# ActiveVisionLab/gaussctrl

Measured on AMD Instinct MI355X. Metric: edited views/sec @512x512 (ControlNet denoise + splat render+bwd), higher is better.
Workload: dtype bf16

## Files before the change

gaussctrl_amd/csrc/dn_gemm_kernels.h:

```cpp
#pragma once
#include "dn_common.h"
#include <type_traits>

namespace dng {
struct GemmArgs {
    int64_t M, N, K;
    const void *A; int64_t lda;
    int B, Hi, Wi, Cin, Ho, Wo, stride, ups, pad;
    const void *W;
    const float *bias;
    const float *rowvec; int64_t ld_rowvec; int64_t rows_per_batch;
    const void *residual; int64_t ldr;
    float out_scale;
    int act, geglu;
    void *out; int64_t ldc; int out_f32;
    void *out_t; int64_t ldt; int64_t t_batch_stride; int64_t t_col0;
    int splits; int tiles_per_split;
    int persist;
    float *ws;
    const void *zeros;
    const float *row_stats; int row_stat_slots; const float *colsum; float ln_eps, ln_inv_k;
    float *out_row_stats;
    float *out_group_stats;
    int gn_groups, gn_cpg;
    const unsigned char *w_scale;
    int a_scale;
    int out_fp8; float out_qscale;
    int dbg;
    float *chan_parts; int cp_nslab; int cp_rows;
    int64_t w_set_rows, w_set_stride;
    int pw;
    int sm_keys;
    int conv_korder;
};

__device__ __forceinline__ void tile_coords(int64_t bid, int nbm, int nbn, int pw, int64_t &mblk, int64_t &nblk)
{
    if (pw <= 0 || pw >= nbn) { mblk = bid / nbn; nblk = bid % nbn; return; }
    const int64_t per = (int64_t)nbm * pw, p = bid / per, within = bid - p * per;
    const int64_t w = (nbn - p * pw) < pw ? (nbn - p * pw) : pw;
    mblk = within / w; nblk = p * pw + within % w;
}
__device__ __forceinline__ void wg_tile(const GemmArgs &g, int nbm, int nbn, int64_t &mblk, int64_t &nblk, int &slice)
{
    const int64_t tiles = gridDim.x, total = tiles * gridDim.y, lin = blockIdx.x + tiles * blockIdx.y;
    const int64_t xcd = lin & 7, qq = total >> 3, rr = total & 7;
    const int64_t L = (xcd < rr ? xcd * (qq + 1) : rr * (qq + 1) + (xcd - rr) * qq) + (lin >> 3);
    slice = (int)(L / tiles);
    tile_coords(L - (int64_t)slice * tiles, nbm, nbn, g.pw, mblk, nblk);
}
}

namespace {
using namespace dn;
using dng::GemmArgs;

template <int I, int N, class F> __device__ __forceinline__ void static_for(F &&f)
{
    if constexpr (I < N) {
        f(std::integral_constant<int, I>{});
        static_for<I + 1, N>(f);
    }
}

constexpr int BM = 128, BK = 64;
constexpr int NT = 256;


constexpr int GS_SLOTS = 20, GS_MAXG = 32;

__device__ __forceinline__ float row16_sum(float v)
{
    v += __builtin_bit_cast(float, __builtin_amdgcn_update_dpp(0, __builtin_bit_cast(int, v), 0x128, 0xf, 0xf, false));
    v += __builtin_bit_cast(float, __builtin_amdgcn_update_dpp(0, __builtin_bit_cast(int, v), 0x124, 0xf, 0xf, false));
    v += __builtin_bit_cast(float, __builtin_amdgcn_update_dpp(0, __builtin_bit_cast(int, v), 0x122, 0xf, 0xf, false));
    v += __builtin_bit_cast(float, __builtin_amdgcn_update_dpp(0, __builtin_bit_cast(int, v), 0x121, 0xf, 0xf, false));
    return v;
}

__device__ __forceinline__ int lds_off(int r, int c) { return r * 128 + ((c ^ ((r >> 1) & 7)) << 4); }

template <class T>
__device__ __forceinline__ void epilogue_store(const GemmArgs &g, int64_t m, int64_t n, int64_t on, float *v, const float *gate, const uint2 *res_pre = nullptr)
{
    const int64_t bidx = g.rowvec ? m / g.rows_per_batch : 0;
    if (g.row_stats) {
        float2 rs = make_float2(0.f, 0.f);
        for (int sl = 0; sl < g.row_stat_slots; ++sl) {
            const float2 t = *reinterpret_cast<const float2 *>(g.row_stats + ((int64_t)sl * g.M + m) * 2);
            rs.x += t.x; rs.y += t.y;
        }
        const float mean = rs.x * g.ln_inv_k, rstd = rsqrtf(fmaxf(rs.y * g.ln_inv_k - mean * mean, 0.f) + g.ln_eps);
#pragma unroll
        for (int r = 0; r < 4; ++r) v[r] = rstd * (v[r] - mean * g.colsum[n + r]);
    }
#pragma unroll
    for (int r = 0; r < 4; ++r) {
        if (g.bias) v[r] += g.bias[n + r];
        if (g.rowvec) v[r] += g.rowvec[bidx * g.ld_rowvec + n + r];
    }
    if (g.geglu) {
#pragma unroll
        for (int r = 0; r < 4; ++r) {
            float gt = gate[r];
            if (g.bias) gt += g.bias[n + 16 + r];
            v[r] = v[r] * gelu_erf(gt);
        }
    }
    if (g.act == 1) {
#pragma unroll
        for (int r = 0; r < 4; ++r) v[r] = silu(v[r]);
    } else if (g.act == 2) {
#pragma unroll
        for (int r = 0; r < 4; ++r) v[r] = fminf(fmaxf(v[r] * 0.5f + 0.5f, 0.f), 1.f);
    }
#pragma unroll
    for (int r = 0; r < 4; ++r) v[r] *= g.out_scale;
    if (g.residual) {
        const uint2 rr = res_pre ? *res_pre : *reinterpret_cast<const uint2 *>((const unsigned char *)g.residual + (m * g.ldr + on) * 2);
        v[0] += T::to_f((unsigned short)(rr.x & 0xffff)); v[1] += T::to_f((unsigned short)(rr.x >> 16));
        v[2] += T::to_f((unsigned short)(rr.y & 0xffff)); v[3] += T::to_f((unsigned short)(rr.y >> 16));
    }
    const bool to_t = g.out_t && on >= g.t_col0;
    const uint2 pk = make_uint2(pack2<T>(v[0], v[1]), pack2<T>(v[2], v[3]));
    if (g.out && !(to_t && g.t_col0 > 0)) {
        if (g.out_f32)
            *reinterpret_cast<float4 *>((float *)g.out + m * g.ldc + on) = make_float4(v[0], v[1], v[2], v[3]);
        else
            *reinterpret_cast<uint2 *>((unsigned char *)g.out + (m * g.ldc + on) * 2) = pk;
    }
    if (to_t) {
        const int64_t b = m / g.rows_per_batch, tok = m - b * g.rows_per_batch;
        unsigned short *o = (unsigned short *)g.out_t + b * g.t_batch_stride + tok;
#pragma unroll
        for (int r = 0; r < 4; ++r) o[(on - g.t_col0 + r) * g.ldt] = T::from_f(v[r]);
    }
    if (!g.out_f32) {
        v[0] = T::to_f((unsigned short)(pk.x & 0xffff)); v[1] = T::to_f((unsigned short)(pk.x >> 16));
        v[2] = T::to_f((unsigned short)(pk.y & 0xffff)); v[3] = T::to_f((unsigned short)(pk.y >> 16));
    }
}

template <int BM>
__device__ __forceinline__ void row_stats_prologue(const GemmArgs &g, int64_t m_base, float *srow)
{
    const int t = threadIdx.x, r = t & 255, half = t >> 8;
    if (t < 2 * BM) srow[t] = 0.f;
    asm volatile("s_waitcnt lgkmcnt(0)" ::: "memory");
    __builtin_amdgcn_s_barrier();
    if (r < BM) {
        const int64_t m = m_base + r < g.M ? m_base + r : g.M - 1;
        const float *rp = g.row_stats + m * 2;
        const int64_t st = g.M * 2;
        float sx = 0.f, sy = 0.f;
        int sl = half;
        for (; sl + 6 < g.row_stat_slots; sl += 8) {
            const float2 a = *reinterpret_cast<const float2 *>(rp + sl * st), b = *reinterpret_cast<const float2 *>(rp + (sl + 2) * st);
            const float2 c = *reinterpret_cast<const float2 *>(rp + (sl + 4) * st), d = *reinterpret_cast<const float2 *>(rp + (sl + 6) * st);
            sx += (a.x + b.x) + (c.x + d.x); sy += (a.y + b.y) + (c.y + d.y);
        }
        for (; sl < g.row_stat_slots; sl += 2) {
            const float2 a = *reinterpret_cast<const float2 *>(rp + sl * st);
            sx += a.x; sy += a.y;
        }
        __hip_atomic_fetch_add(srow + 2 * r, sx, __ATOMIC_RELAXED, __HIP_MEMORY_SCOPE_WORKGROUP);
        __hip_atomic_fetch_add(srow + 2 * r + 1, sy, __ATOMIC_RELAXED, __HIP_MEMORY_SCOPE_WORKGROUP);
    }
    asm volatile("s_waitcnt vmcnt(0) lgkmcnt(0)" ::: "memory");
}

template <class T, int NTW, int MT, int NTHREADS>
__device__ __forceinline__ void wave_epilogue(const GemmArgs &g, f32x4 (&acc)[NTW][MT], int64_t m_base, int64_t m_wave, int64_t n_wave, int lane,
                                              unsigned char *smem, const float *srow = nullptr, int slice = 0)
{
    const int fr = lane & 15, fc = lane >> 4;
    const int64_t n_lane = n_wave + fc * 4;
    if (g.splits > 1) {
#pragma unroll
        for (int mt = 0; mt < MT; ++mt) {
            const int64_t m = m_wave + mt * 16 + fr;
            if (m >= g.M) continue;
#pragma unroll
            for (int nt = 0; nt < NTW; ++nt) {
                const int64_t n = n_lane + nt * 16;
                if (n < g.N)
                    *reinterpret_cast<float4 *>(g.ws + ((int64_t)slice * g.M + m) * g.N + n) =
                        make_float4(acc[nt][mt][0], acc[nt][mt][1], acc[nt][mt][2], acc[nt][mt][3]);
            }
        }
        return;
    }
    if (g.out_group_stats) {
        asm volatile("s_waitcnt lgkmcnt(0)" ::: "memory");
        __builtin_amdgcn_s_barrier();
        for (int idx = threadIdx.x; idx < GS_SLOTS * GS_MAXG * 2; idx += NTHREADS) reinterpret_cast<float *>(smem)[idx] = 0.f;
        asm volatile("s_waitcnt lgkmcnt(0)" ::: "memory");
        __builtin_amdgcn_s_barrier();
    }
    float4 bia[NTW], csm[NTW];
#pragma unroll
    for (int nt = 0; nt < NTW; ++nt) {
        const int64_t n = n_lane + nt * 16;
        bia[nt] = (g.bias && n < g.N) ? *reinterpret_cast<const float4 *>(g.bias + n) : make_float4(0.f, 0.f, 0.f, 0.f);
        csm[nt] = (g.row_stats && n < g.N) ? *reinterpret_cast<const float4 *>(g.colsum + n) : make_float4(0.f, 0.f, 0.f, 0.f);
    }
    uint2 rs_all[MT][NTW];
#pragma unroll
    for (int mt = 0; mt < MT; ++mt) {
        const int64_t m = m_wave + mt * 16 + fr;
        const bool okm = m < g.M;
        const int64_t mc = okm ? m : 0;
#pragma unroll
        for (int nt = 0; nt < NTW; ++nt) {
            const int64_t n = n_lane + nt * 16;
            const bool okn = okm && n < g.N && !(g.geglu && (nt & 1));
            const int64_t on = g.geglu ? (n_wave + nt * 16) / 2 + fc * 4 : n;
            rs_all[mt][nt] = (g.residual && okn) ? *reinterpret_cast<const uint2 *>((const unsigned char *)g.residual + (mc * g.ldr + on) * 2) : make_uint2(0u, 0u);
        }
    }
    const bool want_cs = g.out_group_stats != nullptr;
    float *red = reinterpret_cast<float *>(smem);
    const int64_t b0 = want_cs ? m_base / g.rows_per_batch : 0;
    float cs[NTW][4], css[NTW][4];
#pragma unroll
    for (int nt = 0; nt < NTW; ++nt)
#pragma unroll
        for (int r = 0; r < 4; ++r) { cs[nt][r] = 0.f; css[nt][r] = 0.f; }
    int64_t cs_b = -1;
    auto flush_cs = [&]() __attribute__((always_inline)) {
        float *rb = red + (cs_b - b0) * (GS_MAXG * 2);
#pragma unroll
        for (int nt = 0; nt < NTW; ++nt) {
            const int64_t n = n_lane + nt * 16;
#pragma unroll
            for (int r = 0; r < 4; ++r) {
                const float a = (g.dbg & 4) ? cs[nt][r] : row16_sum(cs[nt][r]), b = (g.dbg & 4) ? css[nt][r] : row16_sum(css[nt][r]);
                if (fr == 0 && n + r < g.N && !(g.dbg & 2)) {
                    const int gi = (int)(n + r) / g.gn_cpg;
                    __hip_atomic_fetch_add(rb + 2 * gi, a, __ATOMIC_RELAXED, __HIP_MEMORY_SCOPE_WORKGROUP);
                    __hip_atomic_fetch_add(rb + 2 * gi + 1, b, __ATOMIC_RELAXED, __HIP_MEMORY_SCOPE_WORKGROUP);
                }
                cs[nt][r] = 0.f; css[nt][r] = 0.f;
            }
        }
    };
#pragma unroll
    for (int mt = 0; mt < MT; ++mt) {
        const int64_t m = m_wave + mt * 16 + fr;
        const int64_t m_tile = m_wave + mt * 16;
        if (m_tile >= g.M) break;
        const bool okm = m < g.M;
        if (want_cs) {
            const int64_t b = m_tile / g.rows_per_batch;
            if (cs_b >= 0 && b != cs_b) flush_cs();
            cs_b = b;
        }
        const uint2 *rs = rs_all[mt];
        float mean = 0.f, rstd = 1.f;
        if (g.row_stats) {
            float sx = 0.f, sy = 0.f;
            if (srow) {
                const float2 t = *reinterpret_cast<const float2 *>(srow + 2 * (okm ? (int)(m - m_base) : 0));
                sx = t.x; sy = t.y;
            } else {
                const float *rp = g.row_stats + (okm ? m : 0) * 2;
                for (int sl = 0; sl < g.row_stat_slots; ++sl) {
                    const float2 t = *reinterpret_cast<const float2 *>(rp + (int64_t)sl * g.M * 2);
                    sx += t.x; sy += t.y;
                }
            }
            mean = sx * g.ln_inv_k;
            rstd = rsqrtf(fmaxf(sy * g.ln_inv_k - mean * mean, 0.f) + g.ln_eps);
        }
        float4 rv[NTW];
        const int64_t bidx = (g.rowvec && okm) ? m / g.rows_per_batch : 0;
#pragma unroll
        for (int nt = 0; nt < NTW; ++nt) {
            const int64_t n = n_lane + nt * 16;
            rv[nt] = (g.rowvec && n < g.N) ? *reinterpret_cast<const float4 *>(g.rowvec + bidx * g.ld_rowvec + n) : make_float4(0.f, 0.f, 0.f, 0.f);
        }
        float rsum = 0.f, rsq = 0.f;
#pragma unroll
        for (int nt = 0; nt < NTW; ++nt) {
            const int64_t n = n_lane + nt * 16;
            if (n >= g.N) continue;
            if (g.geglu && (nt & 1)) continue;
            float a0 = acc[nt][mt][0], a1 = acc[nt][mt][1], a2 = acc[nt][mt][2], a3 = acc[nt][mt][3];
            if (g.row_stats) {
                a0 = rstd * (a0 - mean * csm[nt].x); a1 = rstd * (a1 - mean * csm[nt].y);
                a2 = rstd * (a2 - mean * csm[nt].z); a3 = rstd * (a3 - mean * csm[nt].w);
            }
            float v[4] = {a0 + bia[nt].x + rv[nt].x, a1 + bia[nt].y + rv[nt].y, a2 + bia[nt].z + rv[nt].z, a3 + bia[nt].w + rv[nt].w};
            int64_t on = n;
            if (g.geglu) {
                constexpr int NP = NTW - 1;
                const int np = nt + 1 < NTW ? nt + 1 : NP;
                float g0 = acc[np][mt][0], g1 = acc[np][mt][1], g2 = acc[np][mt][2], g3 = acc[np][mt][3];
                if (g.row_stats) {
                    g0 = rstd * (g0 - mean * csm[np].x); g1 = rstd * (g1 - mean * csm[np].y);
                    g2 = rstd * (g2 - mean * csm[np].z); g3 = rstd * (g3 - mean * csm[np].w);
                }
                v[0] *= gelu_erf(g0 + bia[np].x); v[1] *= gelu_erf(g1 + bia[np].y);
                v[2] *= gelu_erf(g2 + bia[np].z); v[3] *= gelu_erf(g3 + bia[np].w);
                on = (n_wave + nt * 16) / 2 + fc * 4;
            }
            if (g.act == 1) {
#pragma unroll
                for (int r = 0; r < 4; ++r) v[r] = silu(v[r]);
            } else if (g.act == 2) {
#pragma unroll
                for (int r = 0; r < 4; ++r) v[r] = fminf(fmaxf(v[r] * 0.5f + 0.5f, 0.f), 1.f);
            }
#pragma unroll
            for (int r = 0; r < 4; ++r) v[r] *= g.out_scale;
            if (g.residual) {
                v[0] += T::to_f((unsigned short)(rs[nt].x & 0xffff)); v[1] += T::to_f((unsigned short)(rs[nt].x >> 16));
                v[2] += T::to_f((unsigned short)(rs[nt].y & 0xffff)); v[3] += T::to_f((unsigned short)(rs[nt].y >> 16));
// ... 728 lines not shown
                const uint2 pk = make_uint2(pack2<T>(v[0], v[1]), pack2<T>(v[2], v[3]));
                const bool ok = m < g.M && n < g.N;
                if (ok) *reinterpret_cast<uint2 *>((unsigned char *)g.out + (m * g.ldc + n) * 2) = pk;
                if constexpr (CS) pks[mt][nt] = ok ? pk : make_uint2(0u, 0u);
                if constexpr (LNV == 1) {
                    const float w_ = n < g.N ? 1.f : 0.f;
                    const float t0 = w_ * T::to_f((unsigned short)(pk.x & 0xffff)), t1 = w_ * T::to_f((unsigned short)(pk.x >> 16));
                    const float t2 = w_ * T::to_f((unsigned short)(pk.y & 0xffff)), t3 = w_ * T::to_f((unsigned short)(pk.y >> 16));
                    rsum += (t0 + t1) + (t2 + t3); rsq += (t0 * t0 + t1 * t1) + (t2 * t2 + t3 * t3);
                }
            }
            if constexpr (LNV == 1) {
                rsum += __shfl_xor(rsum, 16, 64); rsq += __shfl_xor(rsq, 16, 64);
                rsum += __shfl_xor(rsum, 32, 64); rsq += __shfl_xor(rsq, 32, 64);
                const int64_t slot = (n_base + wn * (16 * NTW)) / (16 * NTW);
                if (fc == 0 && m < g.M && n_base + wn * (16 * NTW) < g.N)
                    *reinterpret_cast<float2 *>(g.out_row_stats + (slot * g.M + m) * 2) = make_float2(rsum, rsq);
            }
        }
        if constexpr (CS) {
            const int64_t m_split = (m_base / g.rows_per_batch + 1) * g.rows_per_batch;
            const int64_t m_end = m_base + BM < g.M ? m_base + BM : g.M;
            const int npass = m_split < m_end ? 2 : 1;
    #pragma unroll 1
            for (int pass = 0; pass < npass; ++pass) {
                float cs[NTW][4], cq[NTW][4];
    #pragma unroll
                for (int nt = 0; nt < NTW; ++nt)
    #pragma unroll
                    for (int r = 0; r < 4; ++r) { cs[nt][r] = 0.f; cq[nt][r] = 0.f; }
    #pragma unroll
                for (int mt = 0; mt < MT; ++mt) {
                    const int64_t m_tile = m_base + wm * (16 * MT) + mt * 16;
                    const float wgt = ((m_tile >= m_split ? 1 : 0) == pass) ? 1.f : 0.f;
    #pragma unroll
                    for (int nt = 0; nt < NTW; ++nt) {
                        const uint2 pk = pks[mt][nt];
                        const float t0 = wgt != 0.f ? T::to_f((unsigned short)(pk.x & 0xffff)) : 0.f, t1 = wgt != 0.f ? T::to_f((unsigned short)(pk.x >> 16)) : 0.f;
                        const float t2 = wgt != 0.f ? T::to_f((unsigned short)(pk.y & 0xffff)) : 0.f, t3 = wgt != 0.f ? T::to_f((unsigned short)(pk.y >> 16)) : 0.f;
                        cs[nt][0] += t0; cq[nt][0] += t0 * t0; cs[nt][1] += t1; cq[nt][1] += t1 * t1;
                        cs[nt][2] += t2; cq[nt][2] += t2 * t2; cs[nt][3] += t3; cq[nt][3] += t3 * t3;
                    }
                }
                float *tb = ctab + (pass * BN + wn * (16 * NTW) + fc * 4) * 2;
    #pragma unroll
                for (int nt = 0; nt < NTW; ++nt)
    #pragma unroll
                    for (int r = 0; r < 4; ++r) {
                        const float sa = row16_sum(cs[nt][r]), sb = row16_sum(cq[nt][r]);
                        if (fr == 0) {
                            __hip_atomic_fetch_add(tb + (nt * 16 + r) * 2, sa, __ATOMIC_RELAXED, __HIP_MEMORY_SCOPE_WORKGROUP);
                            __hip_atomic_fetch_add(tb + (nt * 16 + r) * 2 + 1, sb, __ATOMIC_RELAXED, __HIP_MEMORY_SCOPE_WORKGROUP);
                        }
                    }
            }
            asm volatile("s_waitcnt lgkmcnt(0)" ::: "memory");
            __builtin_amdgcn_s_barrier();
            const int64_t b0 = m_base / g.rows_per_batch;
            const int cpg = g.gn_cpg, G = (int)(g.N / cpg);
            const int n_hi = (int)(n_base + BN < g.N ? n_base + BN : g.N);
            const int g_first = (int)n_base / cpg, ng = (n_hi - 1) / cpg - g_first + 1;
            for (int i = tid; i < 2 * ng; i += 512) {
                const int slot = i >= ng ? 1 : 0, gg = g_first + i - slot * ng;
                if (slot == 1 && !(m_split < m_end)) continue;
                const int c_lo = gg * cpg > (int)n_base ? gg * cpg : (int)n_base, c_hi = (gg + 1) * cpg < n_hi ? (gg + 1) * cpg : n_hi;
                float s1 = 0.f, s2 = 0.f;
                for (int c = c_lo; c < c_hi; ++c) { const float2 t = *reinterpret_cast<const float2 *>(ctab + (slot * BN + c - (int)n_base) * 2); s1 += t.x; s2 += t.y; }
                const int64_t b = b0 + slot;
                const int64_t slab = mblk - (b * g.rows_per_batch) / BM;
                const int half = gg * cpg < (int)n_base ? 1 : 0;
                *reinterpret_cast<float2 *>(g.chan_parts + ((((b * g.cp_nslab + slab) * G + gg) * 2 + half) * 2)) = make_float2(s1, s2);
            }
        }
    } else {
    float4 bia[NTW], csm[LNV == 2 ? NTW : 1];
#pragma unroll
    for (int nt = 0; nt < NTW; ++nt) {
        const int64_t n = n_lane + nt * 16;
        bia[nt] = (g.bias && n < g.N) ? *reinterpret_cast<const float4 *>(g.bias + n) : make_float4(0.f, 0.f, 0.f, 0.f);
        if constexpr (LNV == 2) csm[nt] = n < g.N ? *reinterpret_cast<const float4 *>(g.colsum + n) : make_float4(0.f, 0.f, 0.f, 0.f);
    }
#pragma unroll
    for (int mt = 0; mt < MT; ++mt) {
        const int64_t m = m_base + wm * (16 * MT) + mt * 16 + fr;
        if (m >= g.M) continue;
        if constexpr (LNV == 2) {
            const float2 st = *reinterpret_cast<const float2 *>(srow + 2 * (wm * (16 * MT) + mt * 16 + fr));
            const float mean = st.x * g.ln_inv_k, rstd = rsqrtf(fmaxf(st.y * g.ln_inv_k - mean * mean, 0.f) + g.ln_eps);
#pragma unroll
            for (int nt = 0; nt < NTW; ++nt) {
                acc[nt][mt][0] = rstd * (acc[nt][mt][0] - mean * csm[nt].x); acc[nt][mt][1] = rstd * (acc[nt][mt][1] - mean * csm[nt].y);
                acc[nt][mt][2] = rstd * (acc[nt][mt][2] - mean * csm[nt].z); acc[nt][mt][3] = rstd * (acc[nt][mt][3] - mean * csm[nt].w);
            }
        }
        float4 rv[NTW];
        uint2 rs[NTW];
        const int64_t bidx = g.rowvec ? m / g.rows_per_batch : 0;
#pragma unroll
        for (int nt = 0; nt < NTW; ++nt) {
            const int64_t n = n_lane + nt * 16;
            const bool okn = n < g.N && !(g.geglu && (nt & 1));
            const int64_t on = g.geglu ? (n_base + wn * (16 * NTW) + nt * 16) / 2 + fc * 4 : n;
            rv[nt] = (g.rowvec && n < g.N) ? *reinterpret_cast<const float4 *>(g.rowvec + bidx * g.ld_rowvec + n) : make_float4(0.f, 0.f, 0.f, 0.f);
            rs[nt] = (g.residual && okn) ? *reinterpret_cast<const uint2 *>((const unsigned char *)g.residual + (m * g.ldr + on) * 2) : make_uint2(0u, 0u);
        }
#pragma unroll
        for (int nt = 0; nt < NTW; ++nt) {
            const int64_t n = n_lane + nt * 16;
            if (n >= g.N) continue;
            if (g.geglu && (nt & 1)) continue;
            float v[4] = {acc[nt][mt][0] + bia[nt].x + rv[nt].x, acc[nt][mt][1] + bia[nt].y + rv[nt].y,
                          acc[nt][mt][2] + bia[nt].z + rv[nt].z, acc[nt][mt][3] + bia[nt].w + rv[nt].w};
            int64_t on = n;
            if (g.geglu) {
                constexpr int NP = NTW - 1;
                const int np = nt + 1 < NTW ? nt + 1 : NP;
                v[0] *= gelu_erf(acc[np][mt][0] + bia[np].x); v[1] *= gelu_erf(acc[np][mt][1] + bia[np].y);
                v[2] *= gelu_erf(acc[np][mt][2] + bia[np].z); v[3] *= gelu_erf(acc[np][mt][3] + bia[np].w);
                on = (n_base + wn * (16 * NTW) + nt * 16) / 2 + fc * 4;
            }
            if (g.act == 1) {
#pragma unroll
                for (int r = 0; r < 4; ++r) v[r] = silu(v[r]);
            } else if (g.act == 2) {
#pragma unroll
                for (int r = 0; r < 4; ++r) v[r] = fminf(fmaxf(v[r] * 0.5f + 0.5f, 0.f), 1.f);
            }
#pragma unroll
            for (int r = 0; r < 4; ++r) v[r] *= g.out_scale;
            if (g.residual) {
                v[0] += T::to_f((unsigned short)(rs[nt].x & 0xffff)); v[1] += T::to_f((unsigned short)(rs[nt].x >> 16));
                v[2] += T::to_f((unsigned short)(rs[nt].y & 0xffff)); v[3] += T::to_f((unsigned short)(rs[nt].y >> 16));
            }
            const bool to_t = g.out_t && on >= g.t_col0;
            const uint2 pk = make_uint2(pack2<T>(v[0], v[1]), pack2<T>(v[2], v[3]));
            if (g.out && !(to_t && g.t_col0 > 0)) {
                if (g.out_f32)
                    *reinterpret_cast<float4 *>((float *)g.out + m * g.ldc + on) = make_float4(v[0], v[1], v[2], v[3]);
                else
                    *reinterpret_cast<uint2 *>((unsigned char *)g.out + (m * g.ldc + on) * 2) = pk;
            }
            if (to_t) {
                const int64_t b = m / g.rows_per_batch, tok = m - b * g.rows_per_batch;
                unsigned short *o = (unsigned short *)g.out_t + b * g.t_batch_stride + tok;
#pragma unroll
                for (int r = 0; r < 4; ++r) o[(on - g.t_col0 + r) * g.ldt] = T::from_f(v[r]);
            }
        }
    }
    }
}


template <class T, int NTW, int MT, int LNV = 0>
__global__ __launch_bounds__(512, 1) void k_gemm8p(const GemmArgs g)
{
    static_assert(LNV == 0 || LNV == 2, "persistent kernel: plain or LayerNorm-folded consumer");
    constexpr int BM = 64 * MT, BN = 32 * NTW, STAGE = BM * 128 + BN * 128, NS = 3;
    constexpr int AG = BM / 8, WG = BN / 8, AI = AG / 8, WI = (WG + 7) / 8;
    static_assert(WG % 8 == 0, "every wave issues the same number of W loads");
    constexpr int GRPW = AI + WI;
    extern __shared__ __attribute__((aligned(16))) unsigned char smem[];
    const int tid = threadIdx.x, lane = tid & 63;
    const int wid = __builtin_amdgcn_readfirstlane(tid >> 6);
    const int wm = wid >> 1, wn = wid & 1;
    const int nbn = (int)((g.N + BN - 1) / BN);
    const int64_t ntiles = ((g.M + BM - 1) / BM) * nbn;
    const int nk = (int)(g.K / BK);
    const unsigned lds0 = (unsigned)(size_t)(__attribute__((address_space(3))) unsigned char *)smem;
    float *srow = reinterpret_cast<float *>(smem + NS * STAGE);
    const int lr = lane >> 3, ls = lane & 7;
    const unsigned char *Ab = (const unsigned char *)g.A, *Wb = (const unsigned char *)g.W;
    auto tile_of = [&](int64_t d, int64_t &m_base, int64_t &n_base) __attribute__((always_inline)) {
        const int64_t xcd = d & 7, qq = ntiles >> 3, rr = ntiles & 7;
        const int64_t bid = (xcd < rr ? xcd * (qq + 1) : rr * (qq + 1) + (xcd - rr) * qq) + (d >> 3);
        int64_t mblk, nblk;
        dng::tile_coords(bid, (int)((g.M + BM - 1) / BM), nbn, g.pw, mblk, nblk);
        m_base = mblk * BM; n_base = nblk * BN;
    };
    int a_off[AI], w_off[WI];
    auto set_offsets = [&](int64_t m_base, int64_t n_base) __attribute__((always_inline)) {
#pragma unroll
        for (int i = 0; i < AI; ++i) {
            const int row = (wid + 8 * i) * 8 + lr;
            const int64_t m = m_base + row;
            a_off[i] = (int)(m < g.M ? m : g.M - 1) * (int)g.lda + (ls ^ ((row >> 1) & 7)) * 8;
        }
#pragma unroll
        for (int i = 0; i < WI; ++i) {
            const int row = (wid + 8 * i) * 8 + lr;
            const int64_t n = n_base + row;
            w_off[i] = (int)(n < g.N ? n : g.N - 1) * (int)g.K + (ls ^ ((row >> 1) & 7)) * 8;
        }
    };
    auto issue_a = [&](int kt, int stage, int i) __attribute__((always_inline)) {
        glds16_s(Ab + (size_t)kt * (BK * 2), (unsigned)(a_off[i] * 2), lds0 + stage * STAGE + (unsigned)((wid + 8 * i) * 1024));
    };
    auto issue_w = [&](int kt, int stage, int i) __attribute__((always_inline)) {
        glds16_s(Wb + (size_t)kt * (BK * 2), (unsigned)(w_off[i] * 2), lds0 + stage * STAGE + (unsigned)(BM * 128 + (wid + 8 * i) * 1024));
    };
    auto issue = [&](int kt, int stage) __attribute__((always_inline)) {
#pragma unroll
        for (int i = 0; i < AI; ++i) issue_a(kt, stage, i);
#pragma unroll
        for (int i = 0; i < WI; ++i) issue_w(kt, stage, i);
    };
    const int fr = lane & 15, fc = lane >> 4;
    const int swz = (fr >> 1) & 7;
    const int fx0 = ((fc ^ swz) << 4), fx1 = (((fc + 4) ^ swz) << 4);
    const int aw0 = BM * 128 + (wn * (16 * NTW) + fr) * 128, aa0 = (wm * (16 * MT) + fr) * 128;
    struct Frag { uint4 w[NTW], a[MT]; };
    auto load_frag = [&](Frag &f, int stage, int ks) __attribute__((always_inline)) {
        const unsigned char *sb = smem + stage * STAGE;
        const int fx = ks ? fx1 : fx0;
#pragma unroll
        for (int t = 0; t < NTW; ++t) f.w[t] = *reinterpret_cast<const uint4 *>(sb + aw0 + fx + t * 2048);
#pragma unroll
        for (int t = 0; t < MT; ++t) f.a[t] = *reinterpret_cast<const uint4 *>(sb + aa0 + fx + t * 2048);
    };
    f32x4 acc[NTW][MT];
    constexpr int NMM = NTW * MT, NPC = AI + WI;
    auto block = [&](const Frag &f, Frag &fn, int st_next, int ks_next, bool load_next, int dma_kt, int dma_stage, auto dma_tag) __attribute__((always_inline)) {
        constexpr bool DMA = decltype(dma_tag)::value;
        static_for<0, NMM>([&](auto m_) __attribute__((always_inline)) {
            constexpr int m = decltype(m_)::value, nt = m / MT, mt = m % MT;
            acc[nt][mt] = T::mfma(f.w[nt], f.a[mt], acc[nt][mt]);
            if constexpr (m == 0) {
                __builtin_amdgcn_sched_barrier(0);
                if (load_next) load_frag(fn, st_next, ks_next);
                __builtin_amdgcn_sched_barrier(0);
            } else if constexpr (DMA && m >= 2) {
                static_for<0, NPC>([&](auto p_) __attribute__((always_inline)) {
                    constexpr int pp = decltype(p_)::value;
                    if constexpr (m == 2 + (pp * (NMM - 3)) / NPC) {
                        __builtin_amdgcn_sched_barrier(0);
                        if constexpr (pp < AI) issue_a(dma_kt, dma_stage, pp); else issue_w(dma_kt, dma_stage, pp - AI);
                        __builtin_amdgcn_sched_barrier(0);
                    }
                });
            }
        });
    };
    auto wait_tiles = [&](auto n_) __attribute__((always_inline)) {
        asm volatile("s_waitcnt vmcnt(%0)" ::"n"(decltype(n_)::value * GRPW) : "memory");
    };

    int64_t d = blockIdx.x, m_base, n_base;
    if (d >= ntiles) return;
    tile_of(d, m_base, n_base);
    set_offsets(m_base, n_base);
    issue(0, 0);
    if (nk > 1) issue(1, 1);
    if (nk > 2) issue(2, 2);
    bool first = true;
    for (;;) {
#pragma unroll
        for (int a = 0; a < NTW; ++a)
#pragma unroll
            for (int b = 0; b < MT; ++b) acc[a][b] = f32x4{0.f, 0.f, 0.f, 0.f};
        if (first) { if (nk > 2) wait_tiles(std::integral_constant<int, 2>{}); else if (nk > 1) wait_tiles(std::integral_constant<int, 1>{}); else wait_tiles(std::integral_constant<int, 0>{}); }
        else asm volatile("s_waitcnt vmcnt(0)" ::: "memory");
        first = false;
        __builtin_amdgcn_s_barrier();
        Frag f0, f1;
        load_frag(f0, 0, 0);
        int st = 0, kt = 0;
        for (; kt + 3 < nk; ++kt) {
            const int st1 = st + 1 == NS ? 0 : st + 1;
            block(f0, f1, st, 1, true, 0, 0, std::false_type{});
            wait_tiles(std::integral_constant<int, 1>{});
            asm volatile("s_waitcnt lgkmcnt(0)" ::: "memory");
            __builtin_amdgcn_s_barrier();
            block(f1, f0, st1, 0, true, kt + 3, st, std::true_type{});
            st = st1;
        }
        for (; kt < nk; ++kt) {
            const int st1 = st + 1 == NS ? 0 : st + 1;
            block(f0, f1, st, 1, true, 0, 0, std::false_type{});
            if (kt + 1 < nk) {
                if (kt + 2 < nk) wait_tiles(std::integral_constant<int, 1>{}); else wait_tiles(std::integral_constant<int, 0>{});
                asm volatile("s_waitcnt lgkmcnt(0)" ::: "memory");
                __builtin_amdgcn_s_barrier();
                block(f1, f0, st1, 0, true, 0, 0, std::false_type{});
            } else {
                block(f1, f0, st1, 0, false, 0, 0, std::false_type{});
            }
            st = st1;
        }
        const int64_t cm = m_base, cn = n_base;
        d += gridDim.x;
        const bool more = d < ntiles;
        asm volatile("s_waitcnt lgkmcnt(0)" ::: "memory");
        __builtin_amdgcn_s_barrier();
        if constexpr (LNV == 2) {
            row_stats_prologue<BM>(g, cm, srow);
            __builtin_amdgcn_s_barrier();
        }
        if (more) {
            tile_of(d, m_base, n_base);
            set_offsets(m_base, n_base);
            issue(0, 0);
            if (nk > 1) issue(1, 1);
            if (nk > 2) issue(2, 2);
        }
        {
            const int64_t n_lane = cn + wn * (16 * NTW) + fc * 4;
            float4 bia[NTW], csm[LNV == 2 ? NTW : 1];
#pragma unroll
            for (int nt = 0; nt < NTW; ++nt) {
                const int64_t n = n_lane + nt * 16;
                bia[nt] = (g.bias && n < g.N) ? *reinterpret_cast<const float4 *>(g.bias + n) : make_float4(0.f, 0.f, 0.f, 0.f);
                if constexpr (LNV == 2) csm[nt] = n < g.N ? *reinterpret_cast<const float4 *>(g.colsum + n) : make_float4(0.f, 0.f, 0.f, 0.f);
            }
            float2 st[LNV == 2 ? MT : 1];
            if constexpr (LNV == 2) {
#pragma unroll
                for (int mt = 0; mt < MT; ++mt) st[mt] = *reinterpret_cast<const float2 *>(srow + 2 * (wm * (16 * MT) + mt * 16 + fr));
            }
#pragma unroll
            for (int mt = 0; mt < MT; ++mt) {
                const int64_t m = cm + wm * (16 * MT) + mt * 16 + fr;
                if (m >= g.M) continue;
                if constexpr (LNV == 2) {
                    const float mean = st[mt].x * g.ln_inv_k, rstd = rsqrtf(fmaxf(st[mt].y * g.ln_inv_k - mean * mean, 0.f) + g.ln_eps);
#pragma unroll
                    for (int nt = 0; nt < NTW; ++nt) {
                        acc[nt][mt][0] = rstd * (acc[nt][mt][0] - mean * csm[nt].x); acc[nt][mt][1] = rstd * (acc[nt][mt][1] - mean * csm[nt].y);
                        acc[nt][mt][2] = rstd * (acc[nt][mt][2] - mean * csm[nt].z); acc[nt][mt][3] = rstd * (acc[nt][mt][3] - mean * csm[nt].w);
                    }
                }
#pragma unroll
                for (int nt = 0; nt < NTW; ++nt) {
                    const int64_t n = n_lane + nt * 16;
                    if (n >= g.N) continue;
                    if (g.geglu && (nt & 1)) continue;
                    float v[4] = {acc[nt][mt][0] + bia[nt].x, acc[nt][mt][1] + bia[nt].y, acc[nt][mt][2] + bia[nt].z, acc[nt][mt][3] + bia[nt].w};
                    int64_t on = n;
                    if (g.geglu) {
                        constexpr int NP = NTW - 1;
                        const int np = nt + 1 < NTW ? nt + 1 : NP;
                        v[0] *= gelu_erf(acc[np][mt][0] + bia[np].x); v[1] *= gelu_erf(acc[np][mt][1] + bia[np].y);
                        v[2] *= gelu_erf(acc[np][mt][2] + bia[np].z); v[3] *= gelu_erf(acc[np][mt][3] + bia[np].w);
                        on = (cn + wn * (16 * NTW) + nt * 16) / 2 + fc * 4;
                    }
                    if (g.act == 1) {
#pragma unroll
                        for (int r = 0; r < 4; ++r) v[r] = silu(v[r]);
                    }
#pragma unroll
                    for (int r = 0; r < 4; ++r) v[r] *= g.out_scale;
                    if (g.residual) {
                        const uint2 rs = *reinterpret_cast<const uint2 *>((const unsigned char *)g.residual + (m * g.ldr + on) * 2);
                        v[0] += T::to_f((unsigned short)(rs.x & 0xffff)); v[1] += T::to_f((unsigned short)(rs.x >> 16));
                        v[2] += T::to_f((unsigned short)(rs.y & 0xffff)); v[3] += T::to_f((unsigned short)(rs.y >> 16));
                    }
                    *reinterpret_cast<uint2 *>((unsigned char *)g.out + (m * g.ldc + on) * 2) = make_uint2(pack2<T>(v[0], v[1]), pack2<T>(v[2], v[3]));
                }
            }
        }
        if (!more) break;
    }
}

template <class T, int NTW, int MT, int LNV = 0>
void launch8p(const GemmArgs &g, int nwg, hipStream_t s)
{
    constexpr size_t lds = 3 * (64 * MT * 128 + 32 * NTW * 128) + (LNV == 2 ? 64 * MT * 8 : 0);
    static_assert(lds <= 160 * 1024, "LDS ring");
    static gc::AttrOnce once;
    gc::ensure_dynamic_lds(once, (const void *)k_gemm8p<T, NTW, MT, LNV>, (int)lds);
    hipLaunchKernelGGL((k_gemm8p<T, NTW, MT, LNV>), dim3(nwg), dim3(512), lds, s, g);
}

typedef __attribute__((ext_vector_type(8))) int i32x8;

template <class T, int MODE, int NTW, int MT, bool FUSE, bool CS = false>
__global__ __launch_bounds__(512, 1) void k_gemm8q(const GemmArgs g)
{
    static_assert(MODE == 2 || MODE == 3, "fp8 path: fast conv (2) and aligned linear (3)");
    constexpr int BM = 64 * MT, BN = 32 * NTW, STAGE = BM * 128 + BN * 128, NS = 3;
    constexpr int AG = BM / 8, WG = BN / 8, AI = AG / 8, WI = (WG + 7) / 8;
    constexpr int BKB = 128;
    extern __shared__ __attribute__((aligned(16))) unsigned char smem[];
    const int tid = threadIdx.x, lane = tid & 63;
    const int wid = __builtin_amdgcn_readfirstlane(tid >> 6);
    const int wm = wid >> 1, wn = wid & 1;
    const int nbn = (int)((g.N + BN - 1) / BN);
    int64_t mblk, nblk;
    int slice;
    wg_tile(g, (int)((g.M + BM - 1) / BM), nbn, mblk, nblk, slice);
    const int64_t m_base = mblk * BM, n_base = nblk * BN;
    const int nk_all = (int)(g.K / BKB);
    const int k0 = g.splits > 1 ? slice * g.tiles_per_split : 0;
    const int nk = g.splits > 1 ? (nk_all - k0 < g.tiles_per_split ? nk_all - k0 : g.tiles_per_split) : nk_all;
    const unsigned lds0 = (unsigned)(size_t)(__attribute__((address_space(3))) unsigned char *)smem;
    float *srow = reinterpret_cast<float *>(smem + NS * STAGE);
    if constexpr (FUSE) {
        if (g.row_stats) row_stats_prologue<BM>(g, m_base, srow);
    }
    static_assert(!(FUSE && CS), "one statistics epilogue at a time");
    float *ctab = reinterpret_cast<float *>(smem + NS * STAGE);
    if constexpr (CS) {
        for (int i = tid; i < 4 * BN; i += 512) ctab[i] = 0.f;
    }
    const int lr = lane >> 3, ls = lane & 7;
    int a_off[AI];
    unsigned a_vm[AI];
    const unsigned char *a_ptr[AI];
#pragma unroll
    for (int i = 0; i < AI; ++i) {
        const int row = (wid + 8 * i) * 8 + lr;
        const int ck = ls ^ ((row >> 1) & 7);
        const int64_t m = m_base + row;
        const bool ok = m < g.M;
        a_vm[i] = 0; a_ptr[i] = (const unsigned char *)g.A; a_off[i] = 0;
        if (MODE == 2) {
            const int mm = ok ? (int)m : 0, hw = g.Ho * g.Wo, b = mm / hw, rem = mm - b * hw, oy = rem / g.Wo;
            const int y0 = oy * g.stride - g.pad, x0 = (rem - oy * g.Wo) * g.stride - g.pad;
            a_ptr[i] = (const unsigned char *)g.A + ((int64_t)(b * g.Hi + y0) * g.Wi + x0) * g.Cin + ck * 16;
            unsigned vm = 0;
#pragma unroll
            for (int tp = 0; tp < 9; ++tp) {
                const int yi = y0 + tp / 3, xi = x0 + tp % 3;
                if (ok && (unsigned)yi < (unsigned)g.Hi && (unsigned)xi < (unsigned)g.Wi) vm |= 1u << tp;
            }
            a_vm[i] = vm;
        } else {
            a_off[i] = (int)(m < g.M ? m : g.M - 1) * (int)g.lda + ck * 16;
        }
    }
    int w_off[WI];
#pragma unroll
    for (int i = 0; i < WI; ++i) {
        const int row = (wid + 8 * i) * 8 + lr;
        const int64_t n = n_base + row;
        w_off[i] = (int)(n < g.N ? n : g.N - 1) * (int)g.K + (ls ^ ((row >> 1) & 7)) * 16;
    }
    const unsigned char *Ab = (const unsigned char *)g.A, *Wb = (const unsigned char *)g.W, *Zp = (const unsigned char *)g.zeros;
    const bool tap_inner = MODE == 2 && g.conv_korder != 0;
    const KOrder kord(tap_inner, BKB, g.Cin);
    KCur cur0 = {0, 0};
    if (MODE == 2) cur0 = kord.at(k0, BKB, g.Cin);
    struct TileSrc { int kb, tap, tap_off; unsigned sbase; KCur next; };
    auto issue_begin = [&](int kt, int stage, const KCur c) __attribute__((always_inline)) -> TileSrc {
        TileSrc t;
        t.kb = (k0 + kt) * BKB; t.tap = 0; t.tap_off = 0; t.next = c;
        if (MODE == 2) {
            const int ci = kord.ci(c);
            t.tap = kord.tap(c);
            t.kb = __builtin_amdgcn_readfirstlane(t.tap * g.Cin + ci);
            const int dy = t.tap / 3, dx = t.tap - dy * 3;
            t.tap_off = (dy * g.Wi + dx) * g.Cin + ci;
            t.next = kord.next(c);
        }
        t.sbase = lds0 + stage * STAGE;
        return t;
    };
    auto issue_a = [&](const TileSrc &t, int i) __attribute__((always_inline)) {
        const unsigned dst = t.sbase + (unsigned)((wid + 8 * i) * 1024);
        if (MODE == 3) { glds16_s(Ab + (size_t)t.kb, (unsigned)a_off[i], dst); return; }
        const bool okm = (a_vm[i] >> t.tap) & 1u;
        glds16(okm ? a_ptr[i] + (int64_t)t.tap_off : Zp, dst);
    };
    auto issue_w = [&](const TileSrc &t, int i, bool has) __attribute__((always_inline)) {
        if (has) glds16_s(Wb + (size_t)t.kb, (unsigned)w_off[i], t.sbase + (unsigned)(BM * 128 + (wid + 8 * i) * 1024));
    };
    auto issue = [&](int kt, int stage, const KCur c) __attribute__((always_inline)) -> KCur {
        const TileSrc t = issue_begin(kt, stage, c);
#pragma unroll
        for (int i = 0; i < AI; ++i) issue_a(t, i);
#pragma unroll
        for (int i = 0; i < WI; ++i) issue_w(t, i, wid + 8 * i < WG);
        return t.next;
    };

    f32x4 acc[NTW][MT];
#pragma unroll
    for (int a = 0; a < NTW; ++a)
#pragma unroll
        for (int b = 0; b < MT; ++b) acc[a][b] = f32x4{0.f, 0.f, 0.f, 0.f};
    const int fr = lane & 15, fc = lane >> 4;
    const int swz = (fr >> 1) & 7;
    const int fx0 = ((fc ^ swz) << 4), fx1 = (((fc + 4) ^ swz) << 4);
    const int aw0 = BM * 128 + (wn * (16 * NTW) + fr) * 128, aa0 = (wm * (16 * MT) + fr) * 128;
    typedef __attribute__((ext_vector_type(4))) int i32x4;
    struct Frag { i32x8 w[NTW], a[MT]; };
    auto ld32 = [&](const unsigned char *p0, const unsigned char *p1) __attribute__((always_inline)) -> i32x8 {
        const i32x4 lo = *reinterpret_cast<const i32x4 *>(p0), hi = *reinterpret_cast<const i32x4 *>(p1);
        return __builtin_shufflevector(lo, hi, 0, 1, 2, 3, 4, 5, 6, 7);
    };
    auto load_frag = [&](Frag &f, int stage) __attribute__((always_inline)) {
        const unsigned char *sb = smem + stage * STAGE;
#pragma unroll
        for (int t = 0; t < NTW; ++t) f.w[t] = ld32(sb + aw0 + fx0 + t * 2048, sb + aw0 + fx1 + t * 2048);
#pragma unroll
        for (int t = 0; t < MT; ++t) f.a[t] = ld32(sb + aa0 + fx0 + t * 2048, sb + aa0 + fx1 + t * 2048);
    };
    int sw[NTW];
#pragma unroll
    for (int t = 0; t < NTW; ++t) {
        const int64_t n = n_base + wn * (16 * NTW) + t * 16 + fr;
        sw[t] = g.w_scale[n < g.N ? n : g.N - 1];
    }
    asm volatile("s_waitcnt vmcnt(0)" ::: "memory");
#pragma unroll
    for (int t = 0; t < NTW; ++t) asm volatile("" : "+v"(sw[t]));
    const int sa = g.a_scale;
    constexpr int NMM = NTW * MT, NPC = AI + WI;
    auto block = [&](const Frag &f, Frag &fn, int st_next, bool load_next, const TileSrc &t, auto dma_tag, auto w3_tag) __attribute__((always_inline)) {
        constexpr bool DMA = decltype(dma_tag)::value, W3 = decltype(w3_tag)::value;
        static_for<0, NMM>([&](auto m_) __attribute__((always_inline)) {
            constexpr int m = decltype(m_)::value, nt = m / MT, mt = m % MT;
            acc[nt][mt] = __builtin_amdgcn_mfma_scale_f32_16x16x128_f8f6f4(f.w[nt], f.a[mt], acc[nt][mt], 0, 0, 0, sw[nt], 0, sa);
            if constexpr (m == 0) {
                __builtin_amdgcn_sched_barrier(0);
                if (load_next) load_frag(fn, st_next);
                __builtin_amdgcn_sched_barrier(0);
            } else if constexpr (DMA && m >= 2) {
                static_for<0, NPC>([&](auto p_) __attribute__((always_inline)) {
                    constexpr int pp = decltype(p_)::value;
                    if constexpr (m == 2 + (pp * (NMM - 3)) / NPC) {
                        __builtin_amdgcn_sched_barrier(0);
                        if constexpr (pp < AI) issue_a(t, pp); else issue_w(t, pp - AI, (pp - AI) < WI - 1 || W3 || WG % 8 == 0);
                        __builtin_amdgcn_sched_barrier(0);
// ... 551 lines not shown
```

gaussctrl_amd/csrc/dn_gemm_ln.hip:

```cpp
#include "dn_gemm_kernels.h"

void dn_gemm_launch_ln(const GemmArgs &g, int dtype, int lnv, bool lean, int ntw, int mt8, dim3 grid, hipStream_t s)
{
    if (dtype == DT_BF16) dispatch8ln<BF16>(g, lnv, lean, ntw, mt8, grid, s); else dispatch8ln<F16>(g, lnv, lean, ntw, mt8, grid, s);
}
```

Measured before the change: 11.36.

## Restructure persistent GEMM epilogue: stage bias/colsum/row stats in LDS, specialize flags

```diff
diff --git a/gaussctrl_amd/csrc/dn_gemm_kernels.h b/gaussctrl_amd/csrc/dn_gemm_kernels.h
--- a/gaussctrl_amd/csrc/dn_gemm_kernels.h
+++ b/gaussctrl_amd/csrc/dn_gemm_kernels.h
@@ -141,6 +141,25 @@
     }
 }
 
+__device__ __forceinline__ float2 row_slab_sums(const GemmArgs &g, int64_t m_base, int r, int half)
+{
+    const int64_t m = m_base + r < g.M ? m_base + r : g.M - 1;
+    const float *rp = g.row_stats + m * 2;
+    const int64_t st = g.M * 2;
+    float sx = 0.f, sy = 0.f;
+    int sl = half;
+    for (; sl + 6 < g.row_stat_slots; sl += 8) {
+        const float2 a = *reinterpret_cast<const float2 *>(rp + sl * st), b = *reinterpret_cast<const float2 *>(rp + (sl + 2) * st);
+        const float2 c = *reinterpret_cast<const float2 *>(rp + (sl + 4) * st), d = *reinterpret_cast<const float2 *>(rp + (sl + 6) * st);
+        sx += (a.x + b.x) + (c.x + d.x); sy += (a.y + b.y) + (c.y + d.y);
+    }
+    for (; sl < g.row_stat_slots; sl += 2) {
+        const float2 a = *reinterpret_cast<const float2 *>(rp + sl * st);
+        sx += a.x; sy += a.y;
+    }
+    return make_float2(sx, sy);
+}
+
 template <int BM>
 __device__ __forceinline__ void row_stats_prologue(const GemmArgs &g, int64_t m_base, float *srow)
 {
@@ -149,20 +168,8 @@
     asm volatile("s_waitcnt lgkmcnt(0)" ::: "memory");
     __builtin_amdgcn_s_barrier();
     if (r < BM) {
-        const int64_t m = m_base + r < g.M ? m_base + r : g.M - 1;
-        const float *rp = g.row_stats + m * 2;
-        const int64_t st = g.M * 2;
-        float sx = 0.f, sy = 0.f;
-        int sl = half;
-        for (; sl + 6 < g.row_stat_slots; sl += 8) {
-            const float2 a = *reinterpret_cast<const float2 *>(rp + sl * st), b = *reinterpret_cast<const float2 *>(rp + (sl + 2) * st);
-            const float2 c = *reinterpret_cast<const float2 *>(rp + (sl + 4) * st), d = *reinterpret_cast<const float2 *>(rp + (sl + 6) * st);
-            sx += (a.x + b.x) + (c.x + d.x); sy += (a.y + b.y) + (c.y + d.y);
-        }
-        for (; sl < g.row_stat_slots; sl += 2) {
-            const float2 a = *reinterpret_cast<const float2 *>(rp + sl * st);
-            sx += a.x; sy += a.y;
-        }
+        const float2 s = row_slab_sums(g, m_base, r, half);
+        const float sx = s.x, sy = s.y;
         __hip_atomic_fetch_add(srow + 2 * r, sx, __ATOMIC_RELAXED, __HIP_MEMORY_SCOPE_WORKGROUP);
         __hip_atomic_fetch_add(srow + 2 * r + 1, sy, __ATOMIC_RELAXED, __HIP_MEMORY_SCOPE_WORKGROUP);
     }
@@ -1197,13 +1204,31 @@
 }
 
 
-template <class T, int NTW, int MT, int LNV = 0>
+#ifdef GEMM8P_STAMPS
+__device__ unsigned long long g_p8_stamps[64];
+#define P8_STAMP(i) do { if (blockIdx.x == 37 && tid == 0 && tile_no < 8) g_p8_stamps[tile_no * 8 + (i)] = __builtin_readcyclecounter(); } while (0)
+#else
+#define P8_STAMP(i) do { } while (0)
+#endif
+
+__device__ __forceinline__ float mul_rn(float a, float b)
+{
+    float p = a * b;
+    asm("" : "+v"(p));
+    return p;
+}
+__device__ __forceinline__ float ln_bias_fused(float acc, float mean, float rstd, float cs, float b) { return __builtin_fmaf(rstd, __builtin_fmaf(-mean, cs, acc), b); }
+__device__ __forceinline__ float ln_bias_split(float acc, float mean, float rstd, float cs, float b) { return mul_rn(rstd, __builtin_fmaf(-mean, cs, acc)) + b; }
+
+template <class T, int NTW, int MT, int LNV = 0, bool GEGLU = false>
 __global__ __launch_bounds__(512, 1) void k_gemm8p(const GemmArgs g)
 {
     static_assert(LNV == 0 || LNV == 2, "persistent kernel: plain or LayerNorm-folded consumer");
+    static_assert(!GEGLU || NTW % 2 == 0, "GEGLU pairs n-tiles (nt, nt + 1) inside a wave");
     constexpr int BM = 64 * MT, BN = 32 * NTW, STAGE = BM * 128 + BN * 128, NS = 3;
     constexpr int AG = BM / 8, WG = BN / 8, AI = AG / 8, WI = (WG + 7) / 8;
     static_assert(WG % 8 == 0, "every wave issues the same number of W loads");
+    static_assert(BM <= 256, "row statistics: one thread per (row, slab parity)");
     constexpr int GRPW = AI + WI;
     extern __shared__ __attribute__((aligned(16))) unsigned char smem[];
     const int tid = threadIdx.x, lane = tid & 63;
@@ -1213,7 +1238,8 @@
     const int64_t ntiles = ((g.M + BM - 1) / BM) * nbn;
     const int nk = (int)(g.K / BK);
     const unsigned lds0 = (unsigned)(size_t)(__attribute__((address_space(3))) unsigned char *)smem;
-    float *srow = reinterpret_cast<float *>(smem + NS * STAGE);
+    float *scol = reinterpret_cast<float *>(smem + NS * STAGE);
+    float *srow = scol + 4 * BN;
     const int lr = lane >> 3, ls = lane & 7;
     const unsigned char *Ab = (const unsigned char *)g.A, *Wb = (const unsigned char *)g.W;
     auto tile_of = [&](int64_t d, int64_t &m_base, int64_t &n_base) __attribute__((always_inline)) {
@@ -1224,7 +1250,7 @@
         m_base = mblk * BM; n_base = nblk * BN;
     };
     int a_off[AI], w_off[WI];
-    auto set_offsets = [&](int64_t m_base, int64_t n_base) __attribute__((always_inline)) {
+    auto offsets_of = [&](int64_t m_base, int64_t n_base, int (&a_off)[AI], int (&w_off)[WI]) __attribute__((always_inline)) {
 #pragma unroll
         for (int i = 0; i < AI; ++i) {
             const int row = (wid + 8 * i) * 8 + lr;
@@ -1293,20 +1319,45 @@
     int64_t d = blockIdx.x, m_base, n_base;
     if (d >= ntiles) return;
     tile_of(d, m_base, n_base);
-    set_offsets(m_base, n_base);
+    offsets_of(m_base, n_base, a_off, w_off);
     issue(0, 0);
     if (nk > 1) issue(1, 1);
     if (nk > 2) issue(2, 2);
-    bool first = true;
+    const bool has_b = g.bias != nullptr, has_res = g.residual != nullptr, has_act = g.act == 1, has_scale = g.out_scale != 1.f;
+    int ebuf = 1, sbuf = 1;
+    int64_t m_stats = -1;
+#ifdef GEMM8P_STAMPS
+    int tile_no = 0;
+#endif
     for (;;) {
+        P8_STAMP(0);
+        ebuf ^= 1;
+        const bool col_thread = tid < (LNV == 2 ? 2 : 1) * (BN / 4);
+        const int col_which = tid / (BN / 4), col_c = (tid % (BN / 4)) * 4;
+        float4 col_v = make_float4(0.f, 0.f, 0.f, 0.f);
+        if (col_thread) {
+            const int64_t n = n_base + col_c, nc = n < g.N ? n : g.N - 4;
+            if (col_which) col_v = *reinterpret_cast<const float4 *>(g.colsum + nc); else if (has_b) col_v = *reinterpret_cast<const float4 *>(g.bias + nc);
+        }
+        const int64_t d_next = d + gridDim.x;
+        const bool more = d_next < ntiles;
+        int64_t m_next = 0, n_next = 0;
+        if (more) tile_of(d_next, m_next, n_next);
+        if (col_thread) *reinterpret_cast<float4 *>(scol + (ebuf * 2 + col_which) * BN + col_c) = col_v;
+        if constexpr (LNV == 2) {
+            if (m_base != m_stats) {
+                m_stats = m_base; sbuf ^= 1;
+                const int r = tid & 255, half = tid >> 8;
+                if (r < BM) *reinterpret_cast<float2 *>(srow + ((sbuf * 2 + half) * BM + r) * 2) = row_slab_sums(g, m_base, r, half);
+            }
+        }
+        asm volatile("s_waitcnt vmcnt(0) lgkmcnt(0)" ::: "memory");
+        __builtin_amdgcn_s_barrier();
+        P8_STAMP(1);
 #pragma unroll
         for (int a = 0; a < NTW; ++a)
 #pragma unroll
             for (int b = 0; b < MT; ++b) acc[a][b] = f32x4{0.f, 0.f, 0.f, 0.f};
-        if (first) { if (nk > 2) wait_tiles(std::integral_constant<int, 2>{}); else if (nk > 1) wait_tiles(std::integral_constant<int, 1>{}); else wait_tiles(std::integral_constant<int, 0>{}); }
-        else asm volatile("s_waitcnt vmcnt(0)" ::: "memory");
-        first = false;
-        __builtin_amdgcn_s_barrier();
         Frag f0, f1;
         load_frag(f0, 0, 0);
         int st = 0, kt = 0;
@@ -1332,89 +1383,109 @@
             }
             st = st1;
         }
+        P8_STAMP(2);
         const int64_t cm = m_base, cn = n_base;
-        d += gridDim.x;
-        const bool more = d < ntiles;
+        d = d_next;
         asm volatile("s_waitcnt lgkmcnt(0)" ::: "memory");
         __builtin_amdgcn_s_barrier();
-        if constexpr (LNV == 2) {
-            row_stats_prologue<BM>(g, cm, srow);
-            __builtin_amdgcn_s_barrier();
-        }
+        P8_STAMP(3);
         if (more) {
-            tile_of(d, m_base, n_base);
-            set_offsets(m_base, n_base);
+            m_base = m_next; n_base = n_next;
+            offsets_of(m_base, n_base, a_off, w_off);
             issue(0, 0);
             if (nk > 1) issue(1, 1);
             if (nk > 2) issue(2, 2);
         }
-        {
+        P8_STAMP(4);
+        auto epilogue = [&](auto act_, auto res_, auto scale_) __attribute__((always_inline)) {
+            constexpr bool ACT = decltype(act_)::value, RES = decltype(res_)::value, SCALE = decltype(scale_)::value;
             const int64_t n_lane = cn + wn * (16 * NTW) + fc * 4;
-            float4 bia[NTW], csm[LNV == 2 ? NTW : 1];
-#pragma unroll
-            for (int nt = 0; nt < NTW; ++nt) {
-                const int64_t n = n_lane + nt * 16;
-                bia[nt] = (g.bias && n < g.N) ? *reinterpret_cast<const float4 *>(g.bias + n) : make_float4(0.f, 0.f, 0.f, 0.f);
-                if constexpr (LNV == 2) csm[nt] = n < g.N ? *reinterpret_cast<const float4 *>(g.colsum + n) : make_float4(0.f, 0.f, 0.f, 0.f);
-            }
-            float2 st[LNV == 2 ? MT : 1];
-            if constexpr (LNV == 2) {
-#pragma unroll
-                for (int mt = 0; mt < MT; ++mt) st[mt] = *reinterpret_cast<const float2 *>(srow + 2 * (wm * (16 * MT) + mt * 16 + fr));
-            }
+            float mean[MT], rstd[MT];
 #pragma unroll
             for (int mt = 0; mt < MT; ++mt) {
-                const int64_t m = cm + wm * (16 * MT) + mt * 16 + fr;
-                if (m >= g.M) continue;
+                mean[mt] = 0.f; rstd[mt] = 1.f;
                 if constexpr (LNV == 2) {
-                    const float mean = st[mt].x * g.ln_inv_k, rstd = rsqrtf(fmaxf(st[mt].y * g.ln_inv_k - mean * mean, 0.f) + g.ln_eps);
-#pragma unroll
-                    for (int nt = 0; nt < NTW; ++nt) {
-                        acc[nt][mt][0] = rstd * (acc[nt][mt][0] - mean * csm[nt].x); acc[nt][mt][1] = rstd * (acc[nt][mt][1] - mean * csm[nt].y);
-                        acc[nt][mt][2] = rstd * (acc[nt][mt][2] - mean * csm[nt].z); acc[nt][mt][3] = rstd * (acc[nt][mt][3] - mean * csm[nt].w);
+                    const int row = wm * (16 * MT) + mt * 16 + fr;
+                    const float2 p0 = *reinterpret_cast<const float2 *>(srow + ((sbuf * 2 + 0) * BM + row) * 2);
+                    const float2 p1 = *reinterpret_cast<const float2 *>(srow + ((sbuf * 2 + 1) * BM + row) * 2);
+                    const float sx = p0.x + p1.x, sy = p0.y + p1.y;
+                    mean[mt] = sx * g.ln_inv_k;
+                    rstd[mt] = rsqrtf(fmaxf(sy * g.ln_inv_k - mean[mt] * mean[mt], 0.f) + g.ln_eps);
+                }
+            }
+#pragma unroll
+            for (int nt = 0; nt < NTW; nt += GEGLU ? 2 : 1) {
+                constexpr int NV = GEGLU ? 2 : 1;
+                float bia[NV][4], csm[NV][4];
+#pragma unroll
+                for (int j = 0; j < NV; ++j) {
+                    const int c = wn * (16 * NTW) + (nt + j) * 16 + fc * 4;
+                    const float4 b4 = *reinterpret_cast<const float4 *>(scol + (ebuf * 2 + 0) * BN + c);
+                    bia[j][0] = b4.x; bia[j][1] = b4.y; bia[j][2] = b4.z; bia[j][3] = b4.w;
+                    if constexpr (LNV == 2) {
+                        const float4 c4 = *reinterpret_cast<const float4 *>(scol + (ebuf * 2 + 1) * BN + c);
+                        csm[j][0] = c4.x; csm[j][1] = c4.y; csm[j][2] = c4.z; csm[j][3] = c4.w;
                     }
                 }
-#pragma unroll
-                for (int nt = 0; nt < NTW; ++nt) {
-                    const int64_t n = n_lane + nt * 16;
-                    if (n >= g.N) continue;
-                    if (g.geglu && (nt & 1)) continue;
-                    float v[4] = {acc[nt][mt][0] + bia[nt].x, acc[nt][mt][1] + bia[nt].y, acc[nt][mt][2] + bia[nt].z, acc[nt][mt][3] + bia[nt].w};
-                    int64_t on = n;
-                    if (g.geglu) {
-                        constexpr int NP = NTW - 1;
-                        const int np = nt + 1 < NTW ? nt + 1 : NP;
-                        v[0] *= gelu_erf(acc[np][mt][0] + bia[np].x); v[1] *= gelu_erf(acc[np][mt][1] + bia[np].y);
-                        v[2] *= gelu_erf(acc[np][mt][2] + bia[np].z); v[3] *= gelu_erf(acc[np][mt][3] + bia[np].w);
-                        on = (cn + wn * (16 * NTW) + nt * 16) / 2 + fc * 4;
+                const int64_t n = n_lane + nt * 16;
+                const int64_t on = GEGLU ? (cn + wn * (16 * NTW) + nt * 16) / 2 + fc * 4 : n;
+#pragma unroll
+                for (int mt = 0; mt < MT; ++mt) {
+                    const int64_t m = cm + wm * (16 * MT) + mt * 16 + fr;
+                    const bool ok = m < g.M && n < g.N;
+                    auto biased = [&](int j, int r) __attribute__((always_inline)) {
+                        const float a = acc[nt + j < NTW ? nt + j : nt][mt][r];
+                        if constexpr (LNV == 2)
+                            return ((nt + j) & 1) ? ln_bias_split(a, mean[mt], rstd[mt], csm[j][r], bia[j][r]) : ln_bias_fused(a, mean[mt], rstd[mt], csm[j][r], bia[j][r]);
+                        else
+                            return a + bia[j][r];
+                    };
+                    float v[4];
+#pragma unroll
+                    for (int r = 0; r < 4; ++r) {
+                        v[r] = biased(0, r);
+                        if constexpr (GEGLU) v[r] = mul_rn(v[r], gelu_erf(biased(1, r)));
+                        if constexpr (ACT) v[r] = silu(v[r]);
+                        if constexpr (SCALE) v[r] = mul_rn(v[r], g.out_scale);
                     }
-                    if (g.act == 1) {
-#pragma unroll
-                        for (int r = 0; r < 4; ++r) v[r] = silu(v[r]);
+                    if constexpr (RES) {
+                        uint2 rr = make_uint2(0u, 0u);
+                        if (ok) rr = *reinterpret_cast<const uint2 *>((const unsigned char *)g.residual + (m * g.ldr + on) * 2);
+                        v[0] += T::to_f((unsigned short)(rr.x & 0xffff)); v[1] += T::to_f((unsigned short)(rr.x >> 16));
+                        v[2] += T::to_f((unsigned short)(rr.y & 0xffff)); v[3] += T::to_f((unsigned short)(rr.y >> 16));
                     }
-#pragma unroll
-                    for (int r = 0; r < 4; ++r) v[r] *= g.out_scale;
-                    if (g.residual) {
-                        const uint2 rs = *reinterpret_cast<const uint2 *>((const unsigned char *)g.residual + (m * g.ldr + on) * 2);
-                        v[0] += T::to_f((unsigned short)(rs.x & 0xffff)); v[1] += T::to_f((unsigned short)(rs.x >> 16));
-                        v[2] += T::to_f((unsigned short)(rs.y & 0xffff)); v[3] += T::to_f((unsigned short)(rs.y >> 16));
-                    }
-                    *reinterpret_cast<uint2 *>((unsigned char *)g.out + (m * g.ldc + on) * 2) = make_uint2(pack2<T>(v[0], v[1]), pack2<T>(v[2], v[3]));
+                    if (ok) *reinterpret_cast<uint2 *>((unsigned char *)g.out + (m * g.ldc + on) * 2) = make_uint2(pack2<T>(v[0], v[1]), pack2<T>(v[2], v[3]));
                 }
             }
-        }
+        };
+        const auto with_scale = [&](auto act_, auto res_) __attribute__((always_inline)) {
+            if (has_scale) epilogue(act_, res_, std::true_type{}); else epilogue(act_, res_, std::false_type{});
+        };
+        const auto with_res = [&](auto act_) __attribute__((always_inline)) {
+            if (has_res) with_scale(act_, std::true_type{}); else with_scale(act_, std::false_type{});
+        };
+        if (has_act) with_res(std::true_type{}); else with_res(std::false_type{});
+        P8_STAMP(5);
+#ifdef GEMM8P_STAMPS
+        ++tile_no;
+#endif
         if (!more) break;
     }
 }
 
+template <class T, int NTW, int MT, int LNV, bool GEGLU>
+void launch8p_g(const GemmArgs &g, int nwg, hipStream_t s)
+{
+    constexpr size_t lds = 3 * (64 * MT * 128 + 32 * NTW * 128) + 32 * NTW * 16 + (LNV == 2 ? 64 * MT * 32 : 0);
+    static_assert(lds <= 160 * 1024, "LDS ring");
+    static gc::AttrOnce once;
+    gc::ensure_dynamic_lds(once, (const void *)k_gemm8p<T, NTW, MT, LNV, GEGLU>, (int)lds);
+    hipLaunchKernelGGL((k_gemm8p<T, NTW, MT, LNV, GEGLU>), dim3(nwg), dim3(512), lds, s, g);
+}
 template <class T, int NTW, int MT, int LNV = 0>
 void launch8p(const GemmArgs &g, int nwg, hipStream_t s)
 {
-    constexpr size_t lds = 3 * (64 * MT * 128 + 32 * NTW * 128) + (LNV == 2 ? 64 * MT * 8 : 0);
-    static_assert(lds <= 160 * 1024, "LDS ring");
-    static gc::AttrOnce once;
-    gc::ensure_dynamic_lds(once, (const void *)k_gemm8p<T, NTW, MT, LNV>, (int)lds);
-    hipLaunchKernelGGL((k_gemm8p<T, NTW, MT, LNV>), dim3(nwg), dim3(512), lds, s, g);
+    if (g.geglu) launch8p_g<T, NTW, MT, LNV, true>(g, nwg, s); else launch8p_g<T, NTW, MT, LNV, false>(g, nwg, s);
 }
 
 typedef __attribute__((ext_vector_type(8))) int i32x8;
diff --git a/gaussctrl_amd/csrc/dn_gemm_ln.hip b/gaussctrl_amd/csrc/dn_gemm_ln.hip
--- a/gaussctrl_amd/csrc/dn_gemm_ln.hip
+++ b/gaussctrl_amd/csrc/dn_gemm_ln.hip
@@ -4,3 +4,11 @@
 {
     if (dtype == DT_BF16) dispatch8ln<BF16>(g, lnv, lean, ntw, mt8, grid, s); else dispatch8ln<F16>(g, lnv, lean, ntw, mt8, grid, s);
 }
+
+#ifdef GEMM8P_STAMPS
+extern "C" void gc_dn_gemm8p_stamps(unsigned long long *host64)
+{
+    (void)hipDeviceSynchronize();
+    (void)hipMemcpyFromSymbol(host64, HIP_SYMBOL(g_p8_stamps), sizeof(unsigned long long) * 64);
+}
+#endif
```

After: 11.43, median of 6. About the same (+0.6%).
